# PantoMatrix/PantoMatrix

Hardware: NVIDIA B200
Metric: motion_frames_per_sec (higher is better)
Workload: dtype fp16x3 (two fp16 operand planes, 3 products, f32 accumulate)

## Files before the change

pantomatrix_b200/csrc/pm_tapgemm_tc.cu:

```cuda
#include <cuda.h>
#include <stdio.h>
#include <stdlib.h>

#include <cstring>
#include "pm_common.cuh"
#include "../../include/pm_emage.h"


namespace {

constexpr int BM = 128;
constexpr int BK = 64;
constexpr int UMMA_K = 16;
constexpr int A_TILE_BYTES = BM * BK * 2;
constexpr int NUM_THREADS = 320;
constexpr int MAX_STAGES = 8;
constexpr int OCC2_SMEM_KB = 100;
constexpr int HALO_ROWS = 144;
constexpr int HALO_BYTES = HALO_ROWS * BK * 2;

struct TcParams {
  int taps, pad, nsplit, kblocks;
  int rows_out, cout, batch;
  int R, NB;
  int w_rows;
  const float* bias;
  const float* residual; long long r_bs; int ldr;
  int act, act_cols; float slope;
  float* out_f32; long long o_bs; int ldo;
  __nv_bfloat16* out_bf16; long long ob_ps, ob_bs; int ldob; int out_nsplit;
  int stages;
  const uint8_t* prefetch; long long prefetch_bytes;
  float acc_scale;
  const int* row_limit; int rows_per_clip;
};

#ifdef PM_TC_TIMING
__device__ unsigned long long pm_tc_stamps[4096 * 8];
#define PM_STAMP(i)                                                                                              \
  do {                                                                                                           \
    if ((threadIdx.x & 31) == 0) {                                                                               \
      const unsigned cta_ = (blockIdx.z * gridDim.y + blockIdx.y) * gridDim.x + blockIdx.x;                      \
      if (cta_ < 4096) pm_tc_stamps[cta_ * 8 + (i)] = (unsigned long long)clock64();                             \
    }                                                                                                            \
  } while (0)
#else
#define PM_STAMP(i) do {} while (0)
#endif

#include "pm_tc_ptx.cuh"

__device__ __noinline__ int tc_row_limit(const int* __restrict__ row_limit, int rows_per_clip, int batch, int rows_out,
                                         int b, int l) {
  if (b >= batch || l >= rows_out) return 2;
  int clip = b, r = l;
  if (rows_per_clip > 0) {
    const int g = b * rows_out + l;
    clip = g / rows_per_clip;
    r = g - clip * rows_per_clip;
  }
  const int lim = __ldg(row_limit + clip);
  return r < lim ? 0 : (lim < 0 ? 2 : 1);
}

template <int BN, bool F16, bool CG2, int OCC = 1, bool HALO = false, bool RL = false>
__global__ void __launch_bounds__(NUM_THREADS, OCC) tapgemm_tc_kernel(const __grid_constant__ CUtensorMap map_a,
                                                                    const __grid_constant__ CUtensorMap map_w,
                                                                    const TcParams p) {
  constexpr int W_ROWS_CTA = CG2 ? BN / 2 : BN;
  constexpr int W_TILE_BYTES = W_ROWS_CTA * BK * 2;
  constexpr uint32_t IDESC = (1u << 4) | (F16 ? 0u : ((1u << 7) | (1u << 10))) | ((uint32_t)(BN >> 3) << 17) |
                             ((uint32_t)((CG2 ? 2 * BM : BM) >> 4) << 24);
  constexpr int TMEM_COLS = BN == 64 ? 256 : 512;
  constexpr int ACC = BN;

  extern __shared__ __align__(1024) uint8_t smem_raw[];
  uint8_t* tiles = reinterpret_cast<uint8_t*>((reinterpret_cast<uintptr_t>(smem_raw) + 1023) & ~uintptr_t(1023));
  const int stage_bytes = HALO ? p.nsplit * W_TILE_BYTES : p.nsplit * (A_TILE_BYTES + W_TILE_BYTES);
  uint8_t* ring = HALO ? tiles + p.nsplit * HALO_BYTES : tiles;
  uint64_t* bars = reinterpret_cast<uint64_t*>(ring + (size_t)p.stages * stage_bytes);
  uint64_t* full_bar = bars;
  uint64_t* empty_bar = bars + MAX_STAGES;
  uint64_t* acc_bar = bars + 2 * MAX_STAGES;
  uint32_t* tmem_slot = reinterpret_cast<uint32_t*>(bars + 2 * MAX_STAGES + 1);
  uint64_t* halo_bar = bars + 2 * MAX_STAGES + 2;

  const int warp = threadIdx.x >> 5, lane = threadIdx.x & 31;
  if (warp == 0) PM_STAMP(0);
  const int l0 = blockIdx.x * p.R;
  const int n0 = blockIdx.y * BN;
  const int b0 = blockIdx.z * p.NB;
  const int n_iter = p.taps * p.kblocks;
  const uint32_t cta_rank = CG2 ? cluster_ctarank() : 0u;

  if (warp == 0 && lane == 0) {
    asm volatile("prefetch.tensormap [%0];" ::"l"(&map_a) : "memory");
    asm volatile("prefetch.tensormap [%0];" ::"l"(&map_w) : "memory");
    for (int s = 0; s < p.stages; ++s) {
      mbar_init(smem_u32(&full_bar[s]), 1);
      mbar_init(smem_u32(&empty_bar[s]), 1);
    }
    mbar_init(smem_u32(acc_bar), 1);
    if constexpr (HALO) mbar_init(smem_u32(halo_bar), 1);
    asm volatile("fence.mbarrier_init.release.cluster;" ::: "memory");
  }
  if (warp == 1) {
    if constexpr (CG2) {
      asm volatile("tcgen05.alloc.cta_group::2.sync.aligned.shared::cta.b32 [%0], %1;" ::"r"(smem_u32(tmem_slot)), "n"(TMEM_COLS) : "memory");
      asm volatile("tcgen05.relinquish_alloc_permit.cta_group::2.sync.aligned;" ::: "memory");
    } else {
      asm volatile("tcgen05.alloc.cta_group::1.sync.aligned.shared::cta.b32 [%0], %1;" ::"r"(smem_u32(tmem_slot)), "n"(TMEM_COLS) : "memory");
      asm volatile("tcgen05.relinquish_alloc_permit.cta_group::1.sync.aligned;" ::: "memory");
    }
  }
  tc_fence_before();
  __syncthreads();
  if constexpr (CG2) cluster_sync_all();
  tc_fence_after();
  const uint32_t tmem_base = *tmem_slot;
  if (warp == 0) PM_STAMP(1);

  if (warp == 0) {
    if (lane == 1 && p.prefetch) {
      const long long ncta = (long long)gridDim.x * gridDim.y * gridDim.z;
      const long long cta = ((long long)blockIdx.z * gridDim.y + blockIdx.y) * gridDim.x + blockIdx.x;
      long long share = ((p.prefetch_bytes + ncta - 1) / ncta + 127) & ~127LL;
      long long off = cta * share;
      long long end = off + share < p.prefetch_bytes ? off + share : p.prefetch_bytes;
      end &= ~15LL;
      for (; off < end; off += 16384) {
        const uint32_t n = (uint32_t)(end - off < 16384 ? end - off : 16384);
        asm volatile("cp.async.bulk.prefetch.L2.global [%0], %1;" ::"l"(p.prefetch + off), "r"(n) : "memory");
      }
    }
    if constexpr (HALO) {
      if (elect_one()) {
        mbar_expect_tx(smem_u32(halo_bar), (uint32_t)(p.nsplit * HALO_BYTES));
        for (int pl = 0; pl < p.nsplit; ++pl)
          tma_load_4d(smem_u32(tiles + pl * HALO_BYTES), &map_a, smem_u32(halo_bar), 0, l0 - p.pad, b0, pl);
      }
      __syncwarp();
      int s = 0;
      uint32_t ph = 0;
      for (int it = 0; it < n_iter; ++it) {
        mbar_wait_fast(smem_u32(&empty_bar[s]), ph ^ 1u);
        if (elect_one()) {
          const uint32_t bar = smem_u32(&full_bar[s]);
          mbar_expect_tx(bar, (uint32_t)(p.nsplit * W_TILE_BYTES));
          for (int pl = 0; pl < p.nsplit; ++pl)
            tma_load_3d(smem_u32(ring + (size_t)s * stage_bytes + pl * W_TILE_BYTES), &map_w, bar, 0, it * p.w_rows + n0, pl);
        }
        __syncwarp();
        if (++s == p.stages) { s = 0; ph ^= 1u; }
      }
    } else {
      const uint32_t tx = (uint32_t)(p.nsplit * (A_TILE_BYTES + W_TILE_BYTES));
      int s = 0, tap = 0, kb = 0;
      uint32_t ph = 0;
      for (int it = 0; it < n_iter; ++it) {
        mbar_wait_fast(smem_u32(&empty_bar[s]), ph ^ 1u);
        const uint32_t bar = smem_u32(&full_bar[s]);
        uint8_t* st = tiles + (size_t)s * stage_bytes;
        if (elect_one()) {
        if constexpr (CG2) {
          if (cta_rank == 0) mbar_expect_tx(bar, 2 * tx);
        } else {
          mbar_expect_tx(bar, tx);
        }
        for (int pl = 0; pl < p.nsplit; ++pl) {
          const uint32_t a_dst = smem_u32(st + pl * A_TILE_BYTES);
          const uint32_t w_dst = smem_u32(st + p.nsplit * A_TILE_BYTES + pl * W_TILE_BYTES);
          if constexpr (CG2) {
            tma_load_4d_cg2(a_dst, &map_a, bar, kb * BK, l0 + tap - p.pad, b0, pl);
            tma_load_3d_cg2(w_dst, &map_w, bar, kb * BK, tap * p.w_rows + n0 + (int)cta_rank * W_ROWS_CTA, pl);
          } else {
            tma_load_4d(a_dst, &map_a, bar, kb * BK, l0 + tap - p.pad, b0, pl);
            tma_load_3d(w_dst, &map_w, bar, kb * BK, tap * p.w_rows + n0, pl);
          }
        }
        }
        __syncwarp();
        if (++s == p.stages) { s = 0; ph ^= 1u; }
        if (++kb == p.kblocks) { kb = 0; ++tap; }
      }
    }
  } else if (warp == 1) {
    if (cta_rank == 0)
    {
      const uint64_t desc_hi = (1ull << 16) | ((uint64_t)(1024 >> 4) << 32) | (1ull << 46) | (2ull << 61);
      auto mma = [](uint32_t d, uint64_t a, uint64_t b, uint32_t idesc, uint32_t acc) {
        if constexpr (CG2) tc_mma_cg2(d, a, b, idesc, acc);
        else tc_mma_bf16(d, a, b, idesc, acc);
      };
      auto commit = [](uint32_t bar) {
        if constexpr (CG2) tc_commit_cg2(bar);
        else tc_commit(bar);
      };
      const uint32_t tiles_u32 = smem_u32(tiles);
      const uint32_t ring_u32 = smem_u32(ring);
      const uint32_t d_corr = tmem_base + 2 * ACC;
      if constexpr (HALO) {
        mbar_wait_fast(smem_u32(halo_bar), 0);
        tc_fence_after();
      }
      uint32_t first_main0 = 1, first_main1 = 1, first_corr = 1;
      int s = 0;
      uint32_t ph = 0;
      for (int it = 0; it < n_iter; ++it) {
        mbar_wait_fast(smem_u32(&full_bar[s]), ph);
        tc_fence_after();
        if (it == 0) PM_STAMP(2);
        if (elect_one()) {
        const uint32_t a_base = HALO ? tiles_u32 + (uint32_t)it * 128u
                                     : tiles_u32 + (uint32_t)s * (uint32_t)stage_bytes;
        const uint32_t w_base = HALO ? ring_u32 + (uint32_t)s * (uint32_t)stage_bytes : a_base + p.nsplit * A_TILE_BYTES;
        const uint64_t a0 = desc_hi | (uint64_t)((a_base >> 4) & 0x3FFFu);
        const uint64_t w0 = desc_hi | (uint64_t)((w_base >> 4) & 0x3FFFu);
        constexpr uint64_t A_PL = (HALO ? HALO_BYTES : A_TILE_BYTES) >> 4, W_PL = W_TILE_BYTES >> 4, K_ST = (UMMA_K * 2) >> 4;
        const bool odd = it & 1;
        const uint32_t d_main = tmem_base + (odd ? ACC : 0);
        if (p.nsplit == 3) {
#pragma unroll
          for (int k = 0; k < BK / UMMA_K; ++k) mma(d_corr, a0 + k * K_ST, w0 + 2 * W_PL + k * K_ST, IDESC, (k | (int)(first_corr ^ 1u)) != 0);
#pragma unroll
          for (int k = 0; k < BK / UMMA_K; ++k) mma(d_corr, a0 + A_PL + k * K_ST, w0 + W_PL + k * K_ST, IDESC, 1);
#pragma unroll
          for (int k = 0; k < BK / UMMA_K; ++k) mma(d_corr, a0 + 2 * A_PL + k * K_ST, w0 + k * K_ST, IDESC, 1);
        }
        if (p.nsplit >= 2) {
          const uint32_t fresh = p.nsplit == 3 ? 0u : first_corr;
#pragma unroll
          for (int k = 0; k < BK / UMMA_K; ++k) mma(d_corr, a0 + k * K_ST, w0 + W_PL + k * K_ST, IDESC, (k | (int)(fresh ^ 1u)) != 0);
#pragma unroll
          for (int k = 0; k < BK / UMMA_K; ++k) mma(d_corr, a0 + A_PL + k * K_ST, w0 + k * K_ST, IDESC, 1);
        }
        {
          const uint32_t first = odd ? first_main1 : first_main0;
#pragma unroll
          for (int k = 0; k < BK / UMMA_K; ++k) mma(d_main, a0 + k * K_ST, w0 + k * K_ST, IDESC, (k | (int)(first ^ 1u)) != 0);
        }
        commit(smem_u32(&empty_bar[s]));
        }
        __syncwarp();
        if (p.nsplit >= 2) first_corr = 0;
        if (it & 1) first_main1 = 0; else first_main0 = 0;
        if (++s == p.stages) { s = 0; ph ^= 1u; }
      }
      if (n_iter > 0 && elect_one()) commit(smem_u32(acc_bar));
      PM_STAMP(3);
    }
  } else {
    const int q = warp & 3;
    const int half = (warp - 2) >> 2;
    constexpr int CW = 32;
    constexpr int LPR = CW / 4;
    constexpr int RPI = 32 / LPR;
    constexpr int NIT = 32 / RPI;
    constexpr int ST = CW + 4;
    const uint32_t stage = smem_u32(tiles) + (warp - 2) * 32 * ST * 4;
    const int sub_r = lane / LPR, c4 = (lane % LPR) * 4;
    const int r_shift = 31 - __clz(p.R);
    const bool vec_f = p.out_f32 && ((p.ldo & 3) == 0) && ((reinterpret_cast<uintptr_t>(p.out_f32) & 15) == 0) && ((p.o_bs & 3) == 0);
    const bool vec_r = p.residual && ((p.ldr & 3) == 0) && ((reinterpret_cast<uintptr_t>(p.residual) & 15) == 0) && ((p.r_bs & 3) == 0);
    const bool vec_b = p.out_bf16 && ((p.ldob & 3) == 0) && ((reinterpret_cast<uintptr_t>(p.out_bf16) & 7) == 0) &&
                       ((p.ob_bs & 3) == 0) && ((p.ob_ps & 3) == 0);
    const bool all_vec = (!p.out_f32 || vec_f) && (!p.residual || vec_r) && (!p.out_bf16 || vec_b);
    const float act_slope = p.act == PM_ACT_NONE ? 1.f : (p.act == PM_ACT_RELU ? 0.f : p.slope);
    long long off_f[NIT], off_r[NIT], off_b[NIT];
    uint32_t row_ok = 0;
#pragma unroll
    for (int i = 0; i < NIT; ++i) {
// ... 84 lines not shown
      } else if (n < p.cout) {
#pragma unroll 1
        for (int i = 0; i < NIT; ++i) {
          const int rt = q * 32 + RPI * i + sub_r;
          const int b = b0 + (rt >> r_shift), l = l0 + (rt & (p.R - 1));
          if (RL ? !((row_ok >> i) & 1u) : (b >= p.batch || l >= p.rows_out)) continue;
          const long long of = (long long)b * p.o_bs + (long long)l * p.ldo;
          const long long orr = (long long)b * p.r_bs + (long long)l * p.ldr;
          const PmPlanes P{p.out_bf16 ? p.out_bf16 + (long long)b * p.ob_bs + (long long)l * p.ldob : nullptr,
                           p.ob_ps, p.ldob, p.out_nsplit};
          const uint32_t src = stage + ((RPI * i + sub_r) * ST + c4) * 4;
#pragma unroll 1
          for (int k = 0; k < 4; ++k) {
            if (n + k >= p.cout) break;
            float y;
            asm volatile("ld.shared.f32 %0, [%1];" : "=f"(y) : "r"(src + 4 * k) : "memory");
            y += k == 0 ? bias4.x : (k == 1 ? bias4.y : (k == 2 ? bias4.z : bias4.w));
            if (p.residual) y += p.residual[orr + n + k];
            y = y < 0.f ? (k == 0 ? s0 : (k == 1 ? s1 : (k == 2 ? s2 : s3))) * y : y;
            if (p.out_f32) p.out_f32[of + n + k] = y;
            if (P.ptr) pm_store_planes_t<F16>(P, 0, n + k, y);
          }
        }
      }
    }
  }
  if (RL && p.row_limit && warp >= 2) {
#pragma unroll 1
    for (int rt = warp - 2; rt < BM; rt += 8) {
      const int b = blockIdx.z * p.NB + rt / p.R, l = blockIdx.x * p.R + rt % p.R;
      if (tc_row_limit(p.row_limit, p.rows_per_clip, p.batch, p.rows_out, b, l) != 1) continue;
      const PmPlanes P{p.out_bf16 ? p.out_bf16 + (long long)b * p.ob_bs + (long long)l * p.ldob : nullptr,
                       p.ob_ps, p.ldob, p.out_nsplit};
#pragma unroll 1
      for (int n = blockIdx.y * BN + lane; n < blockIdx.y * BN + BN && n < p.cout; n += 32) {
        if (p.out_f32) p.out_f32[(long long)b * p.o_bs + (long long)l * p.ldo + n] = 0.f;
        if (P.ptr) pm_store_planes_t<F16>(P, 0, n, 0.f);
      }
    }
  }

  if (warp == 2) PM_STAMP(5);
  tc_fence_before();
  __syncthreads();
  if (warp == 0) PM_STAMP(6);
  if constexpr (CG2) cluster_sync_all();
  if (warp == 1) {
    tc_fence_after();
    if constexpr (CG2) asm volatile("tcgen05.dealloc.cta_group::2.sync.aligned.b32 %0, %1;" ::"r"(tmem_base), "n"(TMEM_COLS) : "memory");
    else asm volatile("tcgen05.dealloc.cta_group::1.sync.aligned.b32 %0, %1;" ::"r"(tmem_base), "n"(TMEM_COLS) : "memory");
  }
}

template <bool VEC, bool F16>
__global__ void __launch_bounds__(256) split_bf16_kernel(const float* __restrict__ x, long long x_bs, int ldx, int rows,
                                                         int ch, __nv_bfloat16* __restrict__ out, long long o_ps,
                                                         long long o_bs, int ldo, int nsplit) {
  const int b = blockIdx.y;
  const float* __restrict__ xb = x + (long long)b * x_bs;
  __nv_bfloat16* __restrict__ ob = out + (long long)b * o_bs;
  if (VEC) {
    const int ch4 = ch >> 2;
    const long long total = (long long)rows * ch4;
    for (long long i = (long long)blockIdx.x * blockDim.x + threadIdx.x; i < total; i += (long long)gridDim.x * blockDim.x) {
      const int r = (int)(i / ch4), c4 = (int)(i - (long long)r * ch4);
      const float4 v = *reinterpret_cast<const float4*>(xb + (long long)r * ldx + 4 * c4);
      const PmPlanes P{ob, o_ps, ldo, nsplit};
      pm_store_planes4_t<F16>(P, r, 4 * c4, v);
    }
  } else {
    const long long total = (long long)rows * ch;
    for (long long i = (long long)blockIdx.x * blockDim.x + threadIdx.x; i < total; i += (long long)gridDim.x * blockDim.x) {
      const int r = (int)(i / ch), c = (int)(i - (long long)r * ch);
      const PmPlanes P{ob, o_ps, ldo, nsplit};
      pm_store_planes_t<F16>(P, r, c, xb[(long long)r * ldx + c]);
    }
  }
}

template <int BN, bool F16, bool CG2, int OCC = 1, bool HALO = false, bool RL = false>
int launch(const CUtensorMap& ma, const CUtensorMap& mw, TcParams& p, dim3 grid, cudaStream_t st, int pair_axis = 0) {
  static_assert(OCC == 1 || (BN == 64 && !CG2), "two CTAs per SM: 64-column tiles only (TMEM columns, registers)");
  static_assert(!HALO || (OCC == 2 && BN == 64), "halo mode is built for the 64-column, two-CTAs-per-SM form");
  const int stage_bytes = HALO ? p.nsplit * BN * BK * 2 : p.nsplit * (A_TILE_BYTES + (CG2 ? BN / 2 : BN) * BK * 2);
  const int fixed_bytes = HALO ? p.nsplit * HALO_BYTES : 0;
  static const int env_kb = getenv("PM_TC_SMEM_KB") ? atoi(getenv("PM_TC_SMEM_KB")) : 200;
  int stages = ((OCC == 2 ? OCC2_SMEM_KB : env_kb) * 1024 - fixed_bytes) / stage_bytes;
  if (stages > MAX_STAGES) stages = MAX_STAGES;
  if (stages < 2) return PM_EUNSUPPORTED;
  p.stages = stages;
  const size_t smem = (size_t)fixed_bytes + (size_t)stages * stage_bytes + 1024  + (2 * MAX_STAGES + 3) * sizeof(uint64_t);
  static unsigned long long configured = 0;
  if (pm_first_use_on_device(configured)) {
    cudaError_t e = cudaFuncSetAttribute(tapgemm_tc_kernel<BN, F16, CG2, OCC, HALO, RL>, cudaFuncAttributeMaxDynamicSharedMemorySize, 227 * 1024);
    if (e != cudaSuccess) { configured = 0; return (int)e; }
  }
  if constexpr (CG2) {
    cudaLaunchConfig_t cfg{};
    cfg.gridDim = grid;
    cfg.blockDim = dim3(NUM_THREADS);
    cfg.dynamicSmemBytes = smem;
    cfg.stream = st;
    cudaLaunchAttribute attr[1];
    attr[0].id = cudaLaunchAttributeClusterDimension;
    attr[0].val.clusterDim.x = pair_axis == 0 ? 2 : 1;
    attr[0].val.clusterDim.y = 1;
    attr[0].val.clusterDim.z = pair_axis == 2 ? 2 : 1;
    cfg.attrs = attr;
    cfg.numAttrs = 1;
    const cudaError_t e = cudaLaunchKernelEx(&cfg, tapgemm_tc_kernel<BN, F16, CG2, OCC, HALO, RL>, ma, mw, p);
    return e == cudaSuccess ? PM_OK : (int)e;
  } else {
    tapgemm_tc_kernel<BN, F16, CG2, OCC, HALO, RL><<<grid, NUM_THREADS, smem, st>>>(ma, mw, p);
    PM_LAUNCH_CHECK();
  }
}

template <bool RL>
int dispatch(const CUtensorMap& ma, const CUtensorMap& mw, TcParams& p, dim3 grid, cudaStream_t st, bool halo, bool f16,
             bool cg2, bool occ2, int BNsel, int pair_axis) {
  if (halo) {
    if (f16) return launch<64, true, false, 2, true, RL>(ma, mw, p, grid, st);
    return launch<64, false, false, 2, true, RL>(ma, mw, p, grid, st);
  }
  if (f16) {
    if (cg2) return launch<128, true, true, 1, false, RL>(ma, mw, p, grid, st, pair_axis);
    if (occ2) return launch<64, true, false, 2, false, RL>(ma, mw, p, grid, st);
    if (BNsel == 64) return launch<64, true, false, 1, false, RL>(ma, mw, p, grid, st);
    return launch<128, true, false, 1, false, RL>(ma, mw, p, grid, st);
  }
  if (occ2) return launch<64, false, false, 2, false, RL>(ma, mw, p, grid, st);
  if (BNsel == 64) return launch<64, false, false, 1, false, RL>(ma, mw, p, grid, st);
  return launch<128, false, false, 1, false, RL>(ma, mw, p, grid, st);
}

}

static int tapgemm_tc_run(const uint16_t* A, long long a_ps, long long a_bs, int lda, int batch, int rows_in, int cin,
                          const uint16_t* W, long long w_ps, int w_rows, int ldw, int taps, int pad, int nsplit,
                          const float* bias, int rows_out, int cout,
                          const float* residual, long long r_bs, int ldr,
                          int act, int act_cols, float slope, float acc_scale,
                          float* out_f32, long long o_bs, int ldo,
                          uint16_t* out_bf16, long long ob_ps, long long ob_bs, int ldob, int out_nsplit,
                          const void* prefetch, long long prefetch_bytes, const int* row_limit, int rows_per_clip,
                          void* stream) {
  PM_REQUIRE(A && W && (out_f32 || out_bf16));
  PM_TAKE_FMT(nsplit, f16);
  PM_TAKE_FMT(out_nsplit, out_f16);
  PM_REQUIRE(!out_bf16 || out_f16 == f16);
  PM_REQUIRE(f16 || acc_scale == 1.0f);
  PM_REQUIRE(!prefetch || (prefetch_bytes >= 0 && (reinterpret_cast<uintptr_t>(prefetch) & 15) == 0));
  PM_REQUIRE(batch > 0 && rows_in > 0 && rows_out > 0 && cin > 0 && cout > 0 && taps > 0);
  PM_REQUIRE(nsplit >= 1 && nsplit <= 3 && (!out_bf16 || (out_nsplit >= 1 && out_nsplit <= 3)));
  PM_REQUIRE(act >= PM_ACT_NONE && act <= PM_ACT_LEAKY);
  PM_REQUIRE((reinterpret_cast<uintptr_t>(A) & 15) == 0 && (reinterpret_cast<uintptr_t>(W) & 15) == 0);
  PM_REQUIRE((lda & 7) == 0 && (ldw & 7) == 0 && lda >= cin && ldw >= cin && w_rows >= cout);
  PM_REQUIRE(batch == 1 || (a_bs & 7) == 0);
  PM_REQUIRE(nsplit == 1 || ((a_ps & 7) == 0 && (w_ps & 7) == 0));
  PM_REQUIRE(!out_f32 || ldo >= cout);
  PM_REQUIRE(!out_bf16 || ldob >= cout);
  PM_REQUIRE(!residual || ldr >= cout);

  int R = 128;
  if (rows_out <= 64 && batch > 1) { R = 16; while (R < rows_out) R <<= 1; }
  const int NB = 128 / R;
  int BNsel = cout <= 64 ? 64 : 128;
  PM_REQUIRE(w_rows % BNsel == 0);
  static const bool cg2_on = !(getenv("PM_TC_CG2") && atoi(getenv("PM_TC_CG2")) == 0);
  const int pair_axis = 0;
  const bool cg2 = cg2_on && f16 && nsplit == 2 && BNsel == 128 && R == 128 && pm_cdiv(rows_out, R) % 2 == 0 &&
                   taps * ((cin + BK - 1) / BK) >= 6;

  static const bool halo_on = !(getenv("PM_TC_HALO") && atoi(getenv("PM_TC_HALO")) == 0);
  const bool halo = halo_on && BNsel == 64 && R == 128 && cin <= BK && taps >= 3 && BM + taps - 1 <= HALO_ROWS && nsplit == 2;

  TcParams p;
  p.taps = taps; p.pad = pad; p.nsplit = nsplit; p.kblocks = (cin + BK - 1) / BK;
  p.rows_out = rows_out; p.cout = cout; p.batch = batch; p.R = R; p.NB = NB; p.w_rows = w_rows;
  p.bias = bias; p.residual = residual; p.r_bs = r_bs; p.ldr = ldr;
  p.act = act; p.act_cols = act_cols <= 0 ? cout : act_cols; p.slope = slope;
  p.out_f32 = out_f32; p.o_bs = o_bs; p.ldo = ldo;
  p.out_bf16 = reinterpret_cast<__nv_bfloat16*>(out_bf16); p.ob_ps = ob_ps; p.ob_bs = ob_bs; p.ldob = ldob;
  p.out_nsplit = out_bf16 ? out_nsplit : 0;
  p.stages = 0;
  p.prefetch = static_cast<const uint8_t*>(prefetch);
  p.prefetch_bytes = prefetch ? prefetch_bytes : 0;
  p.acc_scale = acc_scale;
  p.row_limit = row_limit; p.rows_per_clip = rows_per_clip;
  CUtensorMap ma, mw;
  {
    const long long bs_el = batch > 1 ? a_bs : (long long)rows_in * lda;
    const long long ps_el = nsplit > 1 ? a_ps : bs_el * batch;
    cuuint64_t dims[4] = {(cuuint64_t)cin, (cuuint64_t)rows_in, (cuuint64_t)batch, (cuuint64_t)nsplit};
    cuuint64_t strides[3] = {(cuuint64_t)lda * 2, (cuuint64_t)bs_el * 2, (cuuint64_t)ps_el * 2};
    cuuint32_t box[4] = {(cuuint32_t)BK, (cuuint32_t)(halo ? HALO_ROWS : R), (cuuint32_t)NB, 1};
    if (!encode_map(&ma, A, 4, dims, strides, box, f16)) return PM_EBADARG;
  }
  {
    const long long ps_el = nsplit > 1 ? w_ps : (long long)taps * w_rows * ldw;
    cuuint64_t dims[3] = {(cuuint64_t)cin, (cuuint64_t)taps * w_rows, (cuuint64_t)nsplit};
    cuuint64_t strides[2] = {(cuuint64_t)ldw * 2, (cuuint64_t)ps_el * 2};
    cuuint32_t box[3] = {(cuuint32_t)BK, (cuuint32_t)(cg2 ? BNsel / 2 : BNsel), 1};
    if (!encode_map(&mw, W, 3, dims, strides, box, f16)) return PM_EBADARG;
  }
  dim3 grid(pm_cdiv(rows_out, R), pm_cdiv(cout, BNsel), pm_cdiv(batch, NB));
  PM_REQUIRE(grid.z <= 65535 && grid.y <= 65535);
  static const bool occ2_on = !(getenv("PM_TC_OCC2") && atoi(getenv("PM_TC_OCC2")) == 0);
  const bool occ2 = occ2_on && BNsel == 64 && (long long)grid.x * grid.y * grid.z > 2 * 148 &&
                    OCC2_SMEM_KB * 1024 / (nsplit * (A_TILE_BYTES + 64 * BK * 2)) >= 2;
  if (row_limit) return dispatch<true>(ma, mw, p, grid, (cudaStream_t)stream, halo, f16, cg2, occ2, BNsel, pair_axis);
  return dispatch<false>(ma, mw, p, grid, (cudaStream_t)stream, halo, f16, cg2, occ2, BNsel, pair_axis);
}

extern "C" int pm_tapgemm_tc(const uint16_t* A, long long a_ps, long long a_bs, int lda, int batch, int rows_in, int cin,
                             const uint16_t* W, long long w_ps, int w_rows, int ldw, int taps, int pad, int nsplit,
                             const float* bias, int rows_out, int cout,
                             const float* residual, long long r_bs, int ldr,
                             int act, int act_cols, float slope, float acc_scale,
                             float* out_f32, long long o_bs, int ldo,
                             uint16_t* out_bf16, long long ob_ps, long long ob_bs, int ldob, int out_nsplit,
                             const void* prefetch, long long prefetch_bytes, void* stream) {
  return tapgemm_tc_run(A, a_ps, a_bs, lda, batch, rows_in, cin, W, w_ps, w_rows, ldw, taps, pad, nsplit, bias, rows_out,
                        cout, residual, r_bs, ldr, act, act_cols, slope, acc_scale, out_f32, o_bs, ldo, out_bf16, ob_ps,
                        ob_bs, ldob, out_nsplit, prefetch, prefetch_bytes, nullptr, 0, stream);
}

extern "C" int pm_tapgemm_tc_rl(const uint16_t* A, long long a_ps, long long a_bs, int lda, int batch, int rows_in, int cin,
                                const uint16_t* W, long long w_ps, int w_rows, int ldw, int taps, int pad, int nsplit,
                                const float* bias, int rows_out, int cout,
                                const float* residual, long long r_bs, int ldr,
                                int act, int act_cols, float slope, float acc_scale,
                                float* out_f32, long long o_bs, int ldo,
                                uint16_t* out_bf16, long long ob_ps, long long ob_bs, int ldob, int out_nsplit,
                                const void* prefetch, long long prefetch_bytes, const int* row_limit, int rows_per_clip,
                                void* stream) {
  PM_REQUIRE(rows_per_clip >= 0 && (long long)batch * rows_out < (1LL << 31));
  return tapgemm_tc_run(A, a_ps, a_bs, lda, batch, rows_in, cin, W, w_ps, w_rows, ldw, taps, pad, nsplit, bias, rows_out,
                        cout, residual, r_bs, ldr, act, act_cols, slope, acc_scale, out_f32, o_bs, ldo, out_bf16, ob_ps,
                        ob_bs, ldob, out_nsplit, prefetch, prefetch_bytes, row_limit, rows_per_clip, stream);
}

#ifdef PM_TC_TIMING
extern "C" int pm_tc_timing_reset() {
  cudaError_t e = cudaDeviceSynchronize();
  if (e != cudaSuccess) return (int)e;
  void* d = nullptr;
  e = cudaGetSymbolAddress(&d, pm_tc_stamps);
  if (e != cudaSuccess) return (int)e;
  return (int)cudaMemset(d, 0, sizeof(unsigned long long) * 4096 * 8);
}
extern "C" int pm_tc_timing_read(unsigned long long* host) {
  cudaError_t e = cudaDeviceSynchronize();
  if (e != cudaSuccess) return (int)e;
  return (int)cudaMemcpyFromSymbol(host, pm_tc_stamps, sizeof(unsigned long long) * 4096 * 8);
}
#endif

extern "C" int pm_split_bf16(const float* x, long long x_bs, int ldx, int batch, int rows, int ch,
                             uint16_t* out, long long o_ps, long long o_bs, int ldo, int nsplit, void* stream) {
  PM_TAKE_FMT(nsplit, f16);
  PM_REQUIRE(x && out && batch >= 0 && rows >= 0 && ch > 0 && ldx >= ch && ldo >= ch && nsplit >= 1 && nsplit <= 3);
  if ((long long)batch * rows == 0) return PM_OK;
  PM_REQUIRE(batch <= 65535);
  const bool vec = (ch & 3) == 0 && (ldx & 3) == 0 && (x_bs & 3) == 0 && (ldo & 3) == 0 && (o_bs & 3) == 0 &&
// ... 18 lines not shown
```

Before: 517,300.

## Replace two-CTA-per-SM occupancy mode with persistent kernel using double-buffered TMEM accumulators

Removes the OCC=2 and halo template variants of the tap-GEMM kernel and adds a persistent kernel for 64-column tiles. It launches one CTA per SM and loops over tiles, keeping two TMEM accumulator sets and two halo buffers so the next tile's MMA overlaps the previous tile's epilogue. The epilogue also stages results through shared memory. This is meant to hide epilogue and launch-tail cost, but it gives up the latency hiding that two co-resident CTAs provided and makes synchronisation more complex.

Measured after the change: 520,600 (median of 6 runs). About the same (+0.7%).

```diff
diff --git a/pantomatrix_b200/csrc/pm_tapgemm_tc.cu b/pantomatrix_b200/csrc/pm_tapgemm_tc.cu
--- a/pantomatrix_b200/csrc/pm_tapgemm_tc.cu
+++ b/pantomatrix_b200/csrc/pm_tapgemm_tc.cu
@@ -15,9 +15,11 @@
 constexpr int A_TILE_BYTES = BM * BK * 2;
 constexpr int NUM_THREADS = 320;
 constexpr int MAX_STAGES = 8;
-constexpr int OCC2_SMEM_KB = 100;
 constexpr int HALO_ROWS = 144;
 constexpr int HALO_BYTES = HALO_ROWS * BK * 2;
+constexpr int SMEM_MAX = 227 * 1024;
+constexpr int EPI_ST = 36;
+constexpr int EPI_STAGE_BYTES = 8 * 32 * EPI_ST * 4;
 
 struct TcParams {
   int taps, pad, nsplit, kblocks;
@@ -63,8 +65,8 @@
   return r < lim ? 0 : (lim < 0 ? 2 : 1);
 }
 
-template <int BN, bool F16, bool CG2, int OCC = 1, bool HALO = false, bool RL = false>
-__global__ void __launch_bounds__(NUM_THREADS, OCC) tapgemm_tc_kernel(const __grid_constant__ CUtensorMap map_a,
+template <int BN, bool F16, bool CG2, bool RL = false>
+__global__ void __launch_bounds__(NUM_THREADS, 1) tapgemm_tc_kernel(const __grid_constant__ CUtensorMap map_a,
                                                                     const __grid_constant__ CUtensorMap map_w,
                                                                     const TcParams p) {
   constexpr int W_ROWS_CTA = CG2 ? BN / 2 : BN;
@@ -76,14 +78,12 @@
 
   extern __shared__ __align__(1024) uint8_t smem_raw[];
   uint8_t* tiles = reinterpret_cast<uint8_t*>((reinterpret_cast<uintptr_t>(smem_raw) + 1023) & ~uintptr_t(1023));
-  const int stage_bytes = HALO ? p.nsplit * W_TILE_BYTES : p.nsplit * (A_TILE_BYTES + W_TILE_BYTES);
-  uint8_t* ring = HALO ? tiles + p.nsplit * HALO_BYTES : tiles;
-  uint64_t* bars = reinterpret_cast<uint64_t*>(ring + (size_t)p.stages * stage_bytes);
+  const int stage_bytes = p.nsplit * (A_TILE_BYTES + W_TILE_BYTES);
+  uint64_t* bars = reinterpret_cast<uint64_t*>(tiles + (size_t)p.stages * stage_bytes);
   uint64_t* full_bar = bars;
   uint64_t* empty_bar = bars + MAX_STAGES;
   uint64_t* acc_bar = bars + 2 * MAX_STAGES;
   uint32_t* tmem_slot = reinterpret_cast<uint32_t*>(bars + 2 * MAX_STAGES + 1);
-  uint64_t* halo_bar = bars + 2 * MAX_STAGES + 2;
 
   const int warp = threadIdx.x >> 5, lane = threadIdx.x & 31;
   if (warp == 0) PM_STAMP(0);
@@ -101,7 +101,6 @@
       mbar_init(smem_u32(&empty_bar[s]), 1);
     }
     mbar_init(smem_u32(acc_bar), 1);
-    if constexpr (HALO) mbar_init(smem_u32(halo_bar), 1);
     asm volatile("fence.mbarrier_init.release.cluster;" ::: "memory");
   }
   if (warp == 1) {
@@ -133,27 +132,7 @@
         asm volatile("cp.async.bulk.prefetch.L2.global [%0], %1;" ::"l"(p.prefetch + off), "r"(n) : "memory");
       }
     }
-    if constexpr (HALO) {
-      if (elect_one()) {
-        mbar_expect_tx(smem_u32(halo_bar), (uint32_t)(p.nsplit * HALO_BYTES));
-        for (int pl = 0; pl < p.nsplit; ++pl)
-          tma_load_4d(smem_u32(tiles + pl * HALO_BYTES), &map_a, smem_u32(halo_bar), 0, l0 - p.pad, b0, pl);
-      }
-      __syncwarp();
-      int s = 0;
-      uint32_t ph = 0;
-      for (int it = 0; it < n_iter; ++it) {
-        mbar_wait_fast(smem_u32(&empty_bar[s]), ph ^ 1u);
-        if (elect_one()) {
-          const uint32_t bar = smem_u32(&full_bar[s]);
-          mbar_expect_tx(bar, (uint32_t)(p.nsplit * W_TILE_BYTES));
-          for (int pl = 0; pl < p.nsplit; ++pl)
-            tma_load_3d(smem_u32(ring + (size_t)s * stage_bytes + pl * W_TILE_BYTES), &map_w, bar, 0, it * p.w_rows + n0, pl);
-        }
-        __syncwarp();
-        if (++s == p.stages) { s = 0; ph ^= 1u; }
-      }
-    } else {
+    {
       const uint32_t tx = (uint32_t)(p.nsplit * (A_TILE_BYTES + W_TILE_BYTES));
       int s = 0, tap = 0, kb = 0;
       uint32_t ph = 0;
@@ -197,12 +176,7 @@
         else tc_commit(bar);
       };
       const uint32_t tiles_u32 = smem_u32(tiles);
-      const uint32_t ring_u32 = smem_u32(ring);
       const uint32_t d_corr = tmem_base + 2 * ACC;
-      if constexpr (HALO) {
-        mbar_wait_fast(smem_u32(halo_bar), 0);
-        tc_fence_after();
-      }
       uint32_t first_main0 = 1, first_main1 = 1, first_corr = 1;
       int s = 0;
       uint32_t ph = 0;
@@ -211,12 +185,11 @@
         tc_fence_after();
         if (it == 0) PM_STAMP(2);
         if (elect_one()) {
-        const uint32_t a_base = HALO ? tiles_u32 + (uint32_t)it * 128u
-                                     : tiles_u32 + (uint32_t)s * (uint32_t)stage_bytes;
-        const uint32_t w_base = HALO ? ring_u32 + (uint32_t)s * (uint32_t)stage_bytes : a_base + p.nsplit * A_TILE_BYTES;
+        const uint32_t a_base = tiles_u32 + (uint32_t)s * (uint32_t)stage_bytes;
+        const uint32_t w_base = a_base + p.nsplit * A_TILE_BYTES;
         const uint64_t a0 = desc_hi | (uint64_t)((a_base >> 4) & 0x3FFFu);
         const uint64_t w0 = desc_hi | (uint64_t)((w_base >> 4) & 0x3FFFu);
-        constexpr uint64_t A_PL = (HALO ? HALO_BYTES : A_TILE_BYTES) >> 4, W_PL = W_TILE_BYTES >> 4, K_ST = (UMMA_K * 2) >> 4;
+        constexpr uint64_t A_PL = A_TILE_BYTES >> 4, W_PL = W_TILE_BYTES >> 4, K_ST = (UMMA_K * 2) >> 4;
         const bool odd = it & 1;
         const uint32_t d_main = tmem_base + (odd ? ACC : 0);
         if (p.nsplit == 3) {
@@ -407,6 +380,356 @@
   }
 }
 
+template <bool F16, bool HALO, bool RL>
+__global__ void __launch_bounds__(NUM_THREADS, 1) tapgemm_tc_persistent_kernel(const __grid_constant__ CUtensorMap map_a,
+                                                                              const __grid_constant__ CUtensorMap map_w,
+                                                                              const TcParams p, const dim3 tgrid) {
+  constexpr int BN = 64;
+  constexpr int W_TILE_BYTES = BN * BK * 2;
+  constexpr uint32_t IDESC = (1u << 4) | (F16 ? 0u : ((1u << 7) | (1u << 10))) | ((uint32_t)(BN >> 3) << 17) |
+                             ((uint32_t)(BM >> 4) << 24);
+  constexpr int TMEM_COLS = 512;
+  constexpr uint32_t SET_COLS = 256;
+  constexpr int ACC = BN;
+
+  extern __shared__ __align__(1024) uint8_t smem_raw[];
+  uint8_t* tiles = reinterpret_cast<uint8_t*>((reinterpret_cast<uintptr_t>(smem_raw) + 1023) & ~uintptr_t(1023));
+  const int stage_bytes = HALO ? p.nsplit * W_TILE_BYTES : p.nsplit * (A_TILE_BYTES + W_TILE_BYTES);
+  const int halo_buf_bytes = p.nsplit * HALO_BYTES;
+  uint8_t* ring = HALO ? tiles + 2 * halo_buf_bytes : tiles;
+  uint8_t* epi = ring + (size_t)p.stages * stage_bytes;
+  uint64_t* bars = reinterpret_cast<uint64_t*>(epi + EPI_STAGE_BYTES);
+  uint64_t* full_bar = bars;
+  uint64_t* empty_bar = bars + MAX_STAGES;
+  uint64_t* acc_full = bars + 2 * MAX_STAGES;
+  uint64_t* acc_empty = acc_full + 2;
+  uint64_t* halo_full = acc_full + 4;
+  uint64_t* halo_empty = acc_full + 6;
+  uint32_t* tmem_slot = reinterpret_cast<uint32_t*>(acc_full + 8);
+
+  const int warp = threadIdx.x >> 5, lane = threadIdx.x & 31;
+  if (warp == 0) PM_STAMP(0);
+  const int n_tiles = (int)(tgrid.x * tgrid.y * tgrid.z);
+  const int n_iter = p.taps * p.kblocks;
+  auto origin = [&](int t, int& l0, int& n0, int& b0) {
+    const int r = t / (int)tgrid.x;
+    l0 = (t - r * (int)tgrid.x) * p.R;
+    n0 = (r % (int)tgrid.y) * BN;
+    b0 = (r / (int)tgrid.y) * p.NB;
+  };
+
+  if (warp == 0 && lane == 0) {
+    asm volatile("prefetch.tensormap [%0];" ::"l"(&map_a) : "memory");
+    asm volatile("prefetch.tensormap [%0];" ::"l"(&map_w) : "memory");
+    for (int s = 0; s < p.stages; ++s) {
+      mbar_init(smem_u32(&full_bar[s]), 1);
+      mbar_init(smem_u32(&empty_bar[s]), 1);
+    }
+    for (int k = 0; k < 2; ++k) {
+      mbar_init(smem_u32(&acc_full[k]), 1);
+      mbar_init(smem_u32(&acc_empty[k]), 8);
+      mbar_init(smem_u32(&halo_full[k]), 1);
+      mbar_init(smem_u32(&halo_empty[k]), 1);
+    }
+    asm volatile("fence.mbarrier_init.release.cluster;" ::: "memory");
+  }
+  if (warp == 1) {
+    asm volatile("tcgen05.alloc.cta_group::1.sync.aligned.shared::cta.b32 [%0], %1;" ::"r"(smem_u32(tmem_slot)), "n"(TMEM_COLS) : "memory");
+    asm volatile("tcgen05.relinquish_alloc_permit.cta_group::1.sync.aligned;" ::: "memory");
+  }
+  tc_fence_before();
+  __syncthreads();
+  tc_fence_after();
+  const uint32_t tmem_base = *tmem_slot;
+  if (warp == 0) PM_STAMP(1);
+
+  if (warp == 0) {
+    if (lane == 1 && p.prefetch) {
+      const long long share = ((p.prefetch_bytes + gridDim.x - 1) / gridDim.x + 127) & ~127LL;
+      long long off = (long long)blockIdx.x * share;
+      long long end = off + share < p.prefetch_bytes ? off + share : p.prefetch_bytes;
+      end &= ~15LL;
+      for (; off < end; off += 16384) {
+        const uint32_t n = (uint32_t)(end - off < 16384 ? end - off : 16384);
+        asm volatile("cp.async.bulk.prefetch.L2.global [%0], %1;" ::"l"(p.prefetch + off), "r"(n) : "memory");
+      }
+    }
+    const uint32_t tx = (uint32_t)(HALO ? p.nsplit * W_TILE_BYTES : p.nsplit * (A_TILE_BYTES + W_TILE_BYTES));
+    int s = 0;
+    uint32_t ph = 0;
+    int i = 0;
+    for (int t = blockIdx.x; t < n_tiles; t += gridDim.x, ++i) {
+      int l0, n0, b0;
+      origin(t, l0, n0, b0);
+      if constexpr (HALO) {
+        const int hb = i & 1;
+        mbar_wait_fast(smem_u32(&halo_empty[hb]), ((uint32_t)(i >> 1) & 1u) ^ 1u);
+        if (elect_one()) {
+          const uint32_t bar = smem_u32(&halo_full[hb]);
+          mbar_expect_tx(bar, (uint32_t)halo_buf_bytes);
+          for (int pl = 0; pl < p.nsplit; ++pl)
+            tma_load_4d(smem_u32(tiles + hb * halo_buf_bytes + pl * HALO_BYTES), &map_a, bar, 0, l0 - p.pad, b0, pl);
+        }
+        __syncwarp();
+      }
+      int tap = 0, kb = 0;
+      for (int it = 0; it < n_iter; ++it) {
+        mbar_wait_fast(smem_u32(&empty_bar[s]), ph ^ 1u);
+        if (elect_one()) {
+          const uint32_t bar = smem_u32(&full_bar[s]);
+          uint8_t* st = ring + (size_t)s * stage_bytes;
+          mbar_expect_tx(bar, tx);
+          for (int pl = 0; pl < p.nsplit; ++pl) {
+            if constexpr (HALO) {
+              tma_load_3d(smem_u32(st + pl * W_TILE_BYTES), &map_w, bar, 0, it * p.w_rows + n0, pl);
+            } else {
+              tma_load_4d(smem_u32(st + pl * A_TILE_BYTES), &map_a, bar, kb * BK, l0 + tap - p.pad, b0, pl);
+              tma_load_3d(smem_u32(st + p.nsplit * A_TILE_BYTES + pl * W_TILE_BYTES), &map_w, bar, kb * BK,
+                          tap * p.w_rows + n0, pl);
+            }
+          }
+        }
+        __syncwarp();
+        if (++s == p.stages) { s = 0; ph ^= 1u; }
+        if (++kb == p.kblocks) { kb = 0; ++tap; }
+      }
+    }
+  } else if (warp == 1) {
+    const uint64_t desc_hi = (1ull << 16) | ((uint64_t)(1024 >> 4) << 32) | (1ull << 46) | (2ull << 61);
+    const uint32_t tiles_u32 = smem_u32(tiles);
+    const uint32_t ring_u32 = smem_u32(ring);
+    int s = 0;
+    uint32_t ph = 0;
+    int i = 0;
+    for (int t = blockIdx.x; t < n_tiles; t += gridDim.x, ++i) {
+      const int set = i & 1;
+      const uint32_t use_ph = (uint32_t)(i >> 1) & 1u;
+      mbar_wait_fast(smem_u32(&acc_empty[set]), use_ph ^ 1u);
+      tc_fence_after();
+      if constexpr (HALO) {
+        mbar_wait_fast(smem_u32(&halo_full[set]), use_ph);
+        tc_fence_after();
+      }
+      const uint32_t acc_base = tmem_base + (uint32_t)set * SET_COLS;
+      const uint32_t d_corr = acc_base + 2 * ACC;
+      const uint32_t halo_u32 = tiles_u32 + (uint32_t)(set * halo_buf_bytes);
+      uint32_t first_main0 = 1, first_main1 = 1, first_corr = 1;
+      for (int it = 0; it < n_iter; ++it) {
+        mbar_wait_fast(smem_u32(&full_bar[s]), ph);
+        tc_fence_after();
+        if (i == 0 && it == 0) PM_STAMP(2);
+        if (elect_one()) {
+        const uint32_t a_base = HALO ? halo_u32 + (uint32_t)it * 128u
+                                     : ring_u32 + (uint32_t)s * (uint32_t)stage_bytes;
+        const uint32_t w_base = HALO ? ring_u32 + (uint32_t)s * (uint32_t)stage_bytes : a_base + p.nsplit * A_TILE_BYTES;
+        const uint64_t a0 = desc_hi | (uint64_t)((a_base >> 4) & 0x3FFFu);
+        const uint64_t w0 = desc_hi | (uint64_t)((w_base >> 4) & 0x3FFFu);
+        constexpr uint64_t A_PL = (HALO ? HALO_BYTES : A_TILE_BYTES) >> 4, W_PL = W_TILE_BYTES >> 4, K_ST = (UMMA_K * 2) >> 4;
+        const bool odd = it & 1;
+        const uint32_t d_main = acc_base + (odd ? ACC : 0);
+        if (p.nsplit == 3) {
+#pragma unroll
+          for (int k = 0; k < BK / UMMA_K; ++k) tc_mma_bf16(d_corr, a0 + k * K_ST, w0 + 2 * W_PL + k * K_ST, IDESC, (k | (int)(first_corr ^ 1u)) != 0);
+#pragma unroll
+          for (int k = 0; k < BK / UMMA_K; ++k) tc_mma_bf16(d_corr, a0 + A_PL + k * K_ST, w0 + W_PL + k * K_ST, IDESC, 1);
+#pragma unroll
+          for (int k = 0; k < BK / UMMA_K; ++k) tc_mma_bf16(d_corr, a0 + 2 * A_PL + k * K_ST, w0 + k * K_ST, IDESC, 1);
+        }
+        if (p.nsplit >= 2) {
+          const uint32_t fresh = p.nsplit == 3 ? 0u : first_corr;
+#pragma unroll
+          for (int k = 0; k < BK / UMMA_K; ++k) tc_mma_bf16(d_corr, a0 + k * K_ST, w0 + W_PL + k * K_ST, IDESC, (k | (int)(fresh ^ 1u)) != 0);
+#pragma unroll
+          for (int k = 0; k < BK / UMMA_K; ++k) tc_mma_bf16(d_corr, a0 + A_PL + k * K_ST, w0 + k * K_ST, IDESC, 1);
+        }
+        {
+          const uint32_t first = odd ? first_main1 : first_main0;
+#pragma unroll
+          for (int k = 0; k < BK / UMMA_K; ++k) tc_mma_bf16(d_main, a0 + k * K_ST, w0 + k * K_ST, IDESC, (k | (int)(first ^ 1u)) != 0);
+        }
+        tc_commit(smem_u32(&empty_bar[s]));
+        }
+        __syncwarp();
+        if (p.nsplit >= 2) first_corr = 0;
+        if (it & 1) first_main1 = 0; else first_main0 = 0;
+        if (++s == p.stages) { s = 0; ph ^= 1u; }
+      }
+      if (elect_one()) {
+        if constexpr (HALO) tc_commit(smem_u32(&halo_empty[set]));
+        tc_commit(smem_u32(&acc_full[set]));
+      }
+      __syncwarp();
+    }
+    PM_STAMP(3);
+  } else {
+    const int q = warp & 3;
+    const int half = (warp - 2) >> 2;
+    constexpr int CW = 32;
+    constexpr int LPR = CW / 4;
+    constexpr int RPI = 32 / LPR;
+    constexpr int NIT = 32 / RPI;
+    constexpr int ST = EPI_ST;
+    const uint32_t stage = smem_u32(epi) + (warp - 2) * 32 * ST * 4;
+    const int sub_r = lane / LPR, c4 = (lane % LPR) * 4;
+    const int r_shift = 31 - __clz(p.R);
+    const bool vec_f = p.out_f32 && ((p.ldo & 3) == 0) && ((reinterpret_cast<uintptr_t>(p.out_f32) & 15) == 0) && ((p.o_bs & 3) == 0);
+    const bool vec_r = p.residual && ((p.ldr & 3) == 0) && ((reinterpret_cast<uintptr_t>(p.residual) & 15) == 0) && ((p.r_bs & 3) == 0);
+    const bool vec_b = p.out_bf16 && ((p.ldob & 3) == 0) && ((reinterpret_cast<uintptr_t>(p.out_bf16) & 7) == 0) &&
+                       ((p.ob_bs & 3) == 0) && ((p.ob_ps & 3) == 0);
+    const bool all_vec = (!p.out_f32 || vec_f) && (!p.residual || vec_r) && (!p.out_bf16 || vec_b);
+    const float act_slope = p.act == PM_ACT_NONE ? 1.f : (p.act == PM_ACT_RELU ? 0.f : p.slope);
+    const int c0 = half * CW;
+    int i = 0;
+#pragma unroll 1
+    for (int t = blockIdx.x; t < n_tiles; t += gridDim.x, ++i) {
+      const int set = i & 1;
+      int l0, n0, b0;
+      origin(t, l0, n0, b0);
+      long long off_f[NIT], off_r[NIT], off_b[NIT];
+      uint32_t row_ok = 0;
+#pragma unroll
+      for (int k = 0; k < NIT; ++k) {
+        const int rt = q * 32 + RPI * k + sub_r;
+        const int b = b0 + (rt >> r_shift), l = l0 + (rt & (p.R - 1));
+        if (b < p.batch && l < p.rows_out) row_ok |= 1u << k;
+        off_f[k] = (long long)b * p.o_bs + (long long)l * p.ldo;
+        off_r[k] = (long long)b * p.r_bs + (long long)l * p.ldr;
+        off_b[k] = (long long)b * p.ob_bs + (long long)l * p.ldob;
+      }
+      if (RL && p.row_limit) {
+#pragma unroll 1
+        for (int k = 0; k < NIT; ++k)
+          if (tc_row_limit(p.row_limit, p.rows_per_clip, p.batch, p.rows_out, b0 + ((q * 32 + RPI * k + sub_r) >> r_shift),
+                           l0 + ((q * 32 + RPI * k + sub_r) & (p.R - 1))) != 0)
+            row_ok &= ~(1u << k);
+      }
+      uint32_t acc[CW];
+      float v[CW];
+      const uint32_t lane_col = tmem_base + (uint32_t)set * SET_COLS + ((uint32_t)(q * 32) << 16) + (uint32_t)c0;
+      const int nb = n0 + c0;
+      const int n = nb + c4;
+      const bool fast = all_vec && nb + CW <= p.cout;
+      float4 bias4 = make_float4(0.f, 0.f, 0.f, 0.f);
+      if (p.bias) {
+        if (n < p.cout) bias4.x = __ldg(p.bias + n);
+        if (n + 1 < p.cout) bias4.y = __ldg(p.bias + n + 1);
+        if (n + 2 < p.cout) bias4.z = __ldg(p.bias + n + 2);
+        if (n + 3 < p.cout) bias4.w = __ldg(p.bias + n + 3);
+      }
+      float4 rres[NIT];
+      if (fast && p.residual) {
+#pragma unroll
+        for (int k = 0; k < NIT; ++k)
+          rres[k] = ((row_ok >> k) & 1u) ? *reinterpret_cast<const float4*>(p.residual + off_r[k] + n) : make_float4(0.f, 0.f, 0.f, 0.f);
+      }
+      mbar_wait(smem_u32(&acc_full[set]), (uint32_t)(i >> 1) & 1u);
+      tc_fence_after();
+      if (warp == 2 && i == 0) PM_STAMP(4);
+      __syncwarp();
+      tmem_ld(lane_col, acc);
+#pragma unroll
+      for (int j = 0; j < CW; ++j) v[j] = __uint_as_float(acc[j]);
+      if (n_iter > 1) {
+        tmem_ld(lane_col + ACC, acc);
+#pragma unroll
+        for (int j = 0; j < CW; ++j) v[j] += __uint_as_float(acc[j]);
+      }
+      if (p.nsplit > 1) {
+        tmem_ld(lane_col + 2 * ACC, acc);
+#pragma unroll
+        for (int j = 0; j < CW; ++j) v[j] += __uint_as_float(acc[j]);
+      }
+      tc_fence_before();
+      __syncwarp();
+      if (lane == 0) mbar_arrive(smem_u32(&acc_empty[set]));
+      if constexpr (F16) {
+#pragma unroll
+        for (int j = 0; j < CW; ++j) v[j] *= p.acc_scale;
+      }
+      if (nb < p.cout) {
+#pragma unroll
+        for (int j = 0; j < CW / 4; ++j) sts128(stage + (lane * ST + 4 * j) * 4, v[4 * j], v[4 * j + 1], v[4 * j + 2], v[4 * j + 3]);
+        __syncwarp();
+        const float s0 = n < p.act_cols ? act_slope : 1.f, s1 = n + 1 < p.act_cols ? act_slope : 1.f;
+        const float s2 = n + 2 < p.act_cols ? act_slope : 1.f, s3 = n + 3 < p.act_cols ? act_slope : 1.f;
+        if (fast) {
+#pragma unroll
+          for (int k = 0; k < NIT; ++k) {
+            if (!((row_ok >> k) & 1u)) continue;
+            float4 x = lds128(stage + ((RPI * k + sub_r) * ST + c4) * 4);
+            x.x += bias4.x; x.y += bias4.y; x.z += bias4.z; x.w += bias4.w;
+            if (p.residual) {
+              const float4 r = rres[k];
+              x.x += r.x; x.y += r.y; x.z += r.z; x.w += r.w;
+            }
+            x.x = x.x < 0.f ? s0 * x.x : x.x;
+            x.y = x.y < 0.f ? s1 * x.y : x.y;
+            x.z = x.z < 0.f ? s2 * x.z : x.z;
+            x.w = x.w < 0.f ? s3 * x.w : x.w;
+            if (p.out_f32) *reinterpret_cast<float4*>(p.out_f32 + off_f[k] + n) = x;
+            if (p.out_bf16) {
+              const PmPlanes P{p.out_bf16 + off_b[k], p.ob_ps, p.ldob, p.out_nsplit};
+              pm_store_planes4_t<F16>(P, 0, n, x);
+            }
+          }
+        } else if (n < p.cout) {
+#pragma unroll 1
+          for (int k = 0; k < NIT; ++k) {
+            const int rt = q * 32 + RPI * k + sub_r;
+            const int b = b0 + (rt >> r_shift), l = l0 + (rt & (p.R - 1));
+            if (RL ? !((row_ok >> k) & 1u) : (b >= p.batch || l >= p.rows_out)) continue;
+            const long long of = (long long)b * p.o_bs + (long long)l * p.ldo;
+            const long long orr = (long long)b * p.r_bs + (long long)l * p.ldr;
+            const PmPlanes P{p.out_bf16 ? p.out_bf16 + (long long)b * p.ob_bs + (long long)l * p.ldob : nullptr,
+                             p.ob_ps, p.ldob, p.out_nsplit};
+            const uint32_t src = stage + ((RPI * k + sub_r) * ST + c4) * 4;
+#pragma unroll 1
+            for (int e = 0; e < 4; ++e) {
+              if (n + e >= p.cout) break;
+              float y;
+              asm volatile("ld.shared.f32 %0, [%1];" : "=f"(y) : "r"(src + 4 * e) : "memory");
+              y += e == 0 ? bias4.x : (e == 1 ? bias4.y : (e == 2 ? bias4.z : bias4.w));
+              if (p.residual) y += p.residual[orr + n + e];
+              y = y < 0.f ? (e == 0 ? s0 : (e == 1 ? s1 : (e == 2 ? s2 : s3))) * y : y;
+              if (p.out_f32) p.out_f32[of + n + e] = y;
+              if (P.ptr) pm_store_planes_t<F16>(P, 0, n + e, y);
+            }
+          }
+        }
+        __syncwarp();
+      }
+      if (RL && p.row_limit) {
+#pragma unroll 1
+        for (int rt = warp - 2; rt < BM; rt += 8) {
+          const int b = b0 + rt / p.R, l = l0 + rt % p.R;
+          if (tc_row_limit(p.row_limit, p.rows_per_clip, p.batch, p.rows_out, b, l) != 1) continue;
+          const PmPlanes P{p.out_bf16 ? p.out_bf16 + (long long)b * p.ob_bs + (long long)l * p.ldob : nullptr,
+                           p.ob_ps, p.ldob, p.out_nsplit};
+#pragma unroll 1
+          for (int c = n0 + lane; c < n0 + BN && c < p.cout; c += 32) {
+            if (p.out_f32) p.out_f32[(long long)b * p.o_bs + (long long)l * p.ldo + c] = 0.f;
+            if (P.ptr) pm_store_planes_t<F16>(P, 0, c, 0.f);
+          }
+        }
+      }
+    }
+    if (warp == 2) {
+      PM_STAMP(5);
+#ifdef PM_TC_TIMING
+      if (lane == 0 && blockIdx.x < 4096) pm_tc_stamps[blockIdx.x * 8 + 7] = (unsigned long long)i;
+#endif
+    }
+  }
+
+  tc_fence_before();
+  __syncthreads();
+  if (warp == 0) PM_STAMP(6);
+  if (warp == 1) {
+    tc_fence_after();
+    asm volatile("tcgen05.dealloc.cta_group::1.sync.aligned.b32 %0, %1;" ::"r"(tmem_base), "n"(TMEM_COLS) : "memory");
+  }
+}
+
 template <bool VEC, bool F16>
 __global__ void __launch_bounds__(256) split_bf16_kernel(const float* __restrict__ x, long long x_bs, int ldx, int rows,
                                                          int ch, __nv_bfloat16* __restrict__ out, long long o_ps,
@@ -433,21 +756,18 @@
   }
 }
 
-template <int BN, bool F16, bool CG2, int OCC = 1, bool HALO = false, bool RL = false>
+template <int BN, bool F16, bool CG2, bool RL = false>
 int launch(const CUtensorMap& ma, const CUtensorMap& mw, TcParams& p, dim3 grid, cudaStream_t st, int pair_axis = 0) {
-  static_assert(OCC == 1 || (BN == 64 && !CG2), "two CTAs per SM: 64-column tiles only (TMEM columns, registers)");
-  static_assert(!HALO || (OCC == 2 && BN == 64), "halo mode is built for the 64-column, two-CTAs-per-SM form");
-  const int stage_bytes = HALO ? p.nsplit * BN * BK * 2 : p.nsplit * (A_TILE_BYTES + (CG2 ? BN / 2 : BN) * BK * 2);
-  const int fixed_bytes = HALO ? p.nsplit * HALO_BYTES : 0;
+  const int stage_bytes = p.nsplit * (A_TILE_BYTES + (CG2 ? BN / 2 : BN) * BK * 2);
   static const int env_kb = getenv("PM_TC_SMEM_KB") ? atoi(getenv("PM_TC_SMEM_KB")) : 200;
-  int stages = ((OCC == 2 ? OCC2_SMEM_KB : env_kb) * 1024 - fixed_bytes) / stage_bytes;
+  int stages = env_kb * 1024 / stage_bytes;
   if (stages > MAX_STAGES) stages = MAX_STAGES;
   if (stages < 2) return PM_EUNSUPPORTED;
   p.stages = stages;
-  const size_t smem = (size_t)fixed_bytes + (size_t)stages * stage_bytes + 1024  + (2 * MAX_STAGES + 3) * sizeof(uint64_t);
+  const size_t smem = (size_t)stages * stage_bytes + 1024  + (2 * MAX_STAGES + 3) * sizeof(uint64_t);
   static unsigned long long configured = 0;
   if (pm_first_use_on_device(configured)) {
-    cudaError_t e = cudaFuncSetAttribute(tapgemm_tc_kernel<BN, F16, CG2, OCC, HALO, RL>, cudaFuncAttributeMaxDynamicSharedMemorySize, 227 * 1024);
+    cudaError_t e = cudaFuncSetAttribute(tapgemm_tc_kernel<BN, F16, CG2, RL>, cudaFuncAttributeMaxDynamicSharedMemorySize, SMEM_MAX);
     if (e != cudaSuccess) { configured = 0; return (int)e; }
   }
   if constexpr (CG2) {
@@ -463,30 +783,67 @@
     attr[0].val.clusterDim.z = pair_axis == 2 ? 2 : 1;
     cfg.attrs = attr;
     cfg.numAttrs = 1;
-    const cudaError_t e = cudaLaunchKernelEx(&cfg, tapgemm_tc_kernel<BN, F16, CG2, OCC, HALO, RL>, ma, mw, p);
+    const cudaError_t e = cudaLaunchKernelEx(&cfg, tapgemm_tc_kernel<BN, F16, CG2, RL>, ma, mw, p);
     return e == cudaSuccess ? PM_OK : (int)e;
   } else {
-    tapgemm_tc_kernel<BN, F16, CG2, OCC, HALO, RL><<<grid, NUM_THREADS, smem, st>>>(ma, mw, p);
+    tapgemm_tc_kernel<BN, F16, CG2, RL><<<grid, NUM_THREADS, smem, st>>>(ma, mw, p);
     PM_LAUNCH_CHECK();
   }
+}
+
+int sm_count() {
+  static unsigned long long queried = 0;
+  static int count[64];
+  int d = 0;
+  if (cudaGetDevice(&d) != cudaSuccess) return 0;
+  const bool cached = d >= 0 && d < 64;
+  if (pm_first_use_on_device(queried)) {
+    int n = 0;
+    if (cudaDeviceGetAttribute(&n, cudaDevAttrMultiProcessorCount, d) != cudaSuccess) n = 0;
+    if (!cached) return n;
+    if (n <= 0) queried &= ~(1ull << d);
+    count[d] = n;
+  }
+  return count[d];
+}
+
+template <bool F16, bool HALO, bool RL>
+int launch_persistent(const CUtensorMap& ma, const CUtensorMap& mw, TcParams& p, dim3 tiles, cudaStream_t st) {
+  const int stage_bytes = HALO ? p.nsplit * 64 * BK * 2 : p.nsplit * (A_TILE_BYTES + 64 * BK * 2);
+  const int fixed_bytes = (HALO ? 2 * p.nsplit * HALO_BYTES : 0) + EPI_STAGE_BYTES + 1024  +
+                          (2 * MAX_STAGES + 9) * (int)sizeof(uint64_t);
+  int stages = (SMEM_MAX - fixed_bytes) / stage_bytes;
+  if (stages > MAX_STAGES) stages = MAX_STAGES;
+  if (stages < 2) return PM_EUNSUPPORTED;
+  p.stages = stages;
+  const size_t smem = (size_t)fixed_bytes + (size_t)stages * stage_bytes;
+  static unsigned long long configured = 0;
+  if (pm_first_use_on_device(configured)) {
+    cudaError_t e = cudaFuncSetAttribute(tapgemm_tc_persistent_kernel<F16, HALO, RL>, cudaFuncAttributeMaxDynamicSharedMemorySize, SMEM_MAX);
+    if (e != cudaSuccess) { configured = 0; return (int)e; }
+  }
+  const long long n_tiles = (long long)tiles.x * tiles.y * tiles.z;
+  const int sms = sm_count();
+  if (sms <= 0 || n_tiles >= (1LL << 31)) return PM_EUNSUPPORTED;
+  const unsigned ctas = (unsigned)(n_tiles < sms ? n_tiles : sms);
+  tapgemm_tc_persistent_kernel<F16, HALO, RL><<<ctas, NUM_THREADS, smem, st>>>(ma, mw, p, tiles);
+  PM_LAUNCH_CHECK();
 }
 
 template <bool RL>
 int dispatch(const CUtensorMap& ma, const CUtensorMap& mw, TcParams& p, dim3 grid, cudaStream_t st, bool halo, bool f16,
-             bool cg2, bool occ2, int BNsel, int pair_axis) {
-  if (halo) {
-    if (f16) return launch<64, true, false, 2, true, RL>(ma, mw, p, grid, st);
-    return launch<64, false, false, 2, true, RL>(ma, mw, p, grid, st);
+             bool cg2, bool persistent, int BNsel, int pair_axis) {
+  if (persistent) {
+    if (f16) return halo ? launch_persistent<true, true, RL>(ma, mw, p, grid, st) : launch_persistent<true, false, RL>(ma, mw, p, grid, st);
+    return halo ? launch_persistent<false, true, RL>(ma, mw, p, grid, st) : launch_persistent<false, false, RL>(ma, mw, p, grid, st);
   }
   if (f16) {
-    if (cg2) return launch<128, true, true, 1, false, RL>(ma, mw, p, grid, st, pair_axis);
-    if (occ2) return launch<64, true, false, 2, false, RL>(ma, mw, p, grid, st);
-    if (BNsel == 64) return launch<64, true, false, 1, false, RL>(ma, mw, p, grid, st);
-    return launch<128, true, false, 1, false, RL>(ma, mw, p, grid, st);
-  }
-  if (occ2) return launch<64, false, false, 2, false, RL>(ma, mw, p, grid, st);
-  if (BNsel == 64) return launch<64, false, false, 1, false, RL>(ma, mw, p, grid, st);
-  return launch<128, false, false, 1, false, RL>(ma, mw, p, grid, st);
+    if (cg2) return launch<128, true, true, RL>(ma, mw, p, grid, st, pair_axis);
+    if (BNsel == 64) return launch<64, true, false, RL>(ma, mw, p, grid, st);
+    return launch<128, true, false, RL>(ma, mw, p, grid, st);
+  }
+  if (BNsel == 64) return launch<64, false, false, RL>(ma, mw, p, grid, st);
+  return launch<128, false, false, RL>(ma, mw, p, grid, st);
 }
 
 }
@@ -561,11 +918,9 @@
   }
   dim3 grid(pm_cdiv(rows_out, R), pm_cdiv(cout, BNsel), pm_cdiv(batch, NB));
   PM_REQUIRE(grid.z <= 65535 && grid.y <= 65535);
-  static const bool occ2_on = !(getenv("PM_TC_OCC2") && atoi(getenv("PM_TC_OCC2")) == 0);
-  const bool occ2 = occ2_on && BNsel == 64 && (long long)grid.x * grid.y * grid.z > 2 * 148 &&
-                    OCC2_SMEM_KB * 1024 / (nsplit * (A_TILE_BYTES + 64 * BK * 2)) >= 2;
-  if (row_limit) return dispatch<true>(ma, mw, p, grid, (cudaStream_t)stream, halo, f16, cg2, occ2, BNsel, pair_axis);
-  return dispatch<false>(ma, mw, p, grid, (cudaStream_t)stream, halo, f16, cg2, occ2, BNsel, pair_axis);
+  const bool persistent = halo || (BNsel == 64 && (long long)grid.x * grid.y * grid.z > 2 * 148 && nsplit <= 2);
+  if (row_limit) return dispatch<true>(ma, mw, p, grid, (cudaStream_t)stream, halo, f16, cg2, persistent, BNsel, pair_axis);
+  return dispatch<false>(ma, mw, p, grid, (cudaStream_t)stream, halo, f16, cg2, persistent, BNsel, pair_axis);
 }
 
 extern "C" int pm_tapgemm_tc(const uint16_t* A, long long a_ps, long long a_bs, int lda, int batch, int rows_in, int cin,
```
